# KaHIP/KaMinPar

Measured on NVIDIA H100. Metric: lp_edges_per_second, higher is better.
Workload: dtype int32

## Files before the change

kaminpar_b200/csrc/kmp_lp.cu:

```cuda
#include <cuda_runtime.h>

#include <algorithm>
#include <chrono>
#include <cstdio>
#include <cstring>
#include <new>
#include <string>
#include <vector>

#include <cstdlib>
#include <dlfcn.h>
#include <nccl.h>
#include <cub/device/device_radix_sort.cuh>
#include <cub/device/device_scan.cuh>

#include "../../include/kaminpar_b200_contraction.h"
#include "../../include/kaminpar_b200_lp.h"
#include "lp_commit.cuh"
#include "lp_device.cuh"
#include "lp_lowgroup.cuh"
#include "lp_strict.cuh"
#include "lp_sweep.cuh"

using namespace kmp;
// ... 508 lines not shown
      cudaOccupancyMaxActiveBlocksPerMultiprocessor(&per_sm, kernel, T * TEAMS, smem) != cudaSuccess || per_sm < 1) {
    return false;
  }
  h->team_grid[MODE][EW][P64][team_size_index(T)] = static_cast<uint32_t>(sms * per_sm);
  return true;
}

template <int MODE, bool EW, bool P64> bool configure_team_kernels(kmp_lp_handle *h, int sms) {
  cudaFuncSetAttribute(sweep_hub_scatter<MODE, EW, P64>, cudaFuncAttributeMaxDynamicSharedMemorySize, kHubScatterSmem);
  bool ok = configure_team<MODE, EW, P64, 32, 512, 8, !EW>(h, sms) && configure_team<MODE, EW, P64, 128, 2048, 4>(h, sms) &&
            configure_team<MODE, EW, P64, 512, 8192, 1>(h, sms);
  if constexpr (EW) {
    ok = ok && configure_team<MODE, EW, P64, 1024, 16384, 1>(h, sms);
  } else {
    ok = ok && configure_team<MODE, EW, P64, 1024, 32768, 1, true>(h, sms);
  }
  return ok;
}

template <int MODE, bool EW, bool P64> cudaError_t launch_sweep_t(kmp_lp_handle *h, int tier, const SweepArgs &a) {
  if (a.list_size == 0) {
    return cudaSuccess;
  }
  const uint32_t tgrid = capped(h, grid_for(a.list_size, 256));
  switch (tier) {
  case 0:
    sweep_thread<MODE, EW, P64, 8><<<tgrid, 256, 0, h->sweep_stream>>>(a);
    break;
  case 1:
    sweep_thread<MODE, EW, P64, 16><<<tgrid, 256, 0, h->sweep_stream>>>(a);
    break;
  case 2:
    sweep_thread<MODE, EW, P64, 32><<<tgrid, 256, 0, h->sweep_stream>>>(a);
    break;
  case 3:
    launch_team<MODE, EW, P64, 32, 512, 8, !EW>(h, a);
    break;
  case 4:
    launch_team<MODE, EW, P64, 128, 2048, 4>(h, a);
    break;
  case 5:
    launch_team<MODE, EW, P64, 512, 8192, 1>(h, a);
    break;
  case 6:
    if constexpr (EW) {
      launch_team<MODE, EW, P64, 1024, 16384, 1>(h, a);
    } else {
      launch_team<MODE, EW, P64, 1024, 32768, 1, true>(h, a);
    }
    break;
  default: {
    HubArgs hb{};
    const uint32_t s_idx = h->cur_subround;
    const uint32_t S = h->lists_S;
    const uint32_t first = h->list_off[kHubTier * S + s_idx] - h->list_off[kHubTier * S];
    hb.table_off = h->t4_table_off.p + first;
    hb.g_tab = h->hub_tab.p;
    hb.cursor = h->hub_cursor.p;
    hb.ovf = h->hub_ovf.p;
    hb.ovf_cap = static_cast<uint32_t>(std::min<uint64_t>(h->t4_max_wave_edges, 0xFFFFFFFFull));
    hb.bucket_cap = h->hub_bucket_cap;
    hb.sel_limit = h->hub_sel_limit;
    hb.stage_adjncy = h->adjncy_16b ? 1u : 0u;
    hb.rank = h->rank;
    hb.world = h->world;
    hb.sel_begin = h->t4_sel_begin.p + first;
    hb.hit = h->t4_hit.p + first;
    for (uint32_t w = h->t4_wave_off[s_idx]; w < h->t4_wave_off[s_idx + 1]; ++w) {
      const kmp_lp_handle::HubWave &wv = h->t4_waves[w];
      hb.item_entry = h->t4_item_entry.p + wv.item_lo;
      hb.item_chunk = h->t4_item_chunk.p + wv.item_lo;
      hb.item_u = h->t4_item_u.p + wv.item_lo;
      hb.item_beg = h->t4_item_beg.p + wv.item_lo;
      hb.item_deg = h->t4_item_deg.p + wv.item_lo;
      hb.num_items = wv.item_hi - wv.item_lo;
      hb.queue = h->ctr32.p + 64 + w;
      hb.ovf_count = h->ctr32.p + 512 + w;
      sweep_hub_scatter<MODE, EW, P64><<<capped(h, std::min<uint32_t>(hb.num_items, kSMs * 4)), kHubThreads, kHubScatterSmem, h->sweep_stream>>>(a, hb, h->m);
      hb.sel_entry = h->t4_sel_entry.p + wv.sel_lo;
      hb.sel_piece = h->t4_sel_piece.p + wv.sel_lo;
      hb.num_sel_items = wv.sel_hi - wv.sel_lo;
      hb.part_best = h->t4_part_best.p + (wv.sel_lo - h->t4_sel_off[s_idx]);
      hb.part_fav = h->t4_part_fav.p + (wv.sel_lo - h->t4_sel_off[s_idx]);
      sweep_hub_select<MODE><<<capped(h, std::min<uint32_t>((hb.num_sel_items + kSelWarps - 1) / kSelWarps, kSMs * 6)), kSelWarps * 32, 0, h->sweep_stream>>>(a, hb);
      h->kernel_launches += 2;
    }
    hb.part_best = h->t4_part_best.p;
    hb.part_fav = h->t4_part_fav.p;
    sweep_hub_final<MODE><<<capped(h, grid_for(static_cast<uint64_t>(a.list_size) * 32, 256)), 256, 0, h->sweep_stream>>>(a, hb);
    break;
  }
  }
  return cudaGetLastError();
}

int timed_begin(kmp_lp_handle *h, int tag, cudaStream_t st = nullptr) {
  if (!h->timing) {
    return -1;
  }
  if (st == nullptr) {
    st = h->stream;
  }
  if (h->sweep_events_used == h->sweep_events.size()) {
    cudaEvent_t x, y;
    cudaEventCreate(&x);
    cudaEventCreate(&y);
    h->sweep_events.emplace_back(x, y);
    h->sweep_event_group.push_back(0);
  }
  const int idx = static_cast<int>(h->sweep_events_used++);
  h->sweep_event_group[idx] = tag;
  cudaEventRecord(h->sweep_events[idx].first, st);
  return idx;
}
void timed_end(kmp_lp_handle *h, int idx, cudaStream_t st = nullptr) {
  if (idx >= 0) {
    cudaEventRecord(h->sweep_events[idx].second, st == nullptr ? h->stream : st);
  }
}

cudaError_t launch_sweep(kmp_lp_handle *h, int mode, int tier, const SweepArgs &a_in) {
  if (a_in.list_size == 0) {
    return cudaSuccess;
  }
  SweepArgs a = a_in;
  a.counters = h->ctr64.p + tier;
  a.queue = h->queue.p + static_cast<size_t>(tier) * kNumGroups * h->lists_S + h->cur_sg;
  if (h->sweep_stream == nullptr) {
    h->sweep_stream = h->stream;
  }
  const int ev = timed_begin(h, tier, h->sweep_stream);
  const bool ew = h->adjwgt != nullptr;
  const int variant = (mode << 2) | (ew ? 2 : 0) | (h->p64 ? 1 : 0);
  cudaError_t e;
  switch (variant) {
  case 0: e = launch_sweep_t<0, false, false>(h, tier, a); break;
  case 1: e = launch_sweep_t<0, false, true>(h, tier, a); break;
  case 2: e = launch_sweep_t<0, true, false>(h, tier, a); break;
  case 3: e = launch_sweep_t<0, true, true>(h, tier, a); break;
  case 4: e = launch_sweep_t<1, false, false>(h, tier, a); break;
  case 5: e = launch_sweep_t<1, false, true>(h, tier, a); break;
  case 6: e = launch_sweep_t<1, true, false>(h, tier, a); break;
  default: e = launch_sweep_t<1, true, true>(h, tier, a); break;
  }
  timed_end(h, ev, h->sweep_stream);
  ++h->kernel_launches;
  ++h->sweep_launches;
  ++h->group_launches[tier];
  return e;
}

struct TraceClock {
  bool on = std::getenv("KMP_TRACE") != nullptr;
  std::chrono::steady_clock::time_point t = std::chrono::steady_clock::now();
  void lap(const char *what) {
    if (on) {
      const auto now = std::chrono::steady_clock::now();
      std::fprintf(stderr, "[kmp trace] %-28s %8.3f ms\n", what, std::chrono::duration<double, std::milli>(now - t).count());
      t = now;
    }
  }
};

int ensure_lists(kmp_lp_handle *h) {
  TraceClock tc;
  const uint32_t S = std::max<uint32_t>(1, h->cfg.sync_subrounds);
  if (h->lists_valid && h->lists_S == S && h->lists_G == h->cfg.sync_granule_log2 &&
// ... 1052 lines not shown
  if (mode == 0) {
    cfg->impl = KMP_LP_TWO_PHASE;
    cfg->two_hop_strategy = KMP_TWO_HOP_MATCH_THREADWISE;
    cfg->isolated_nodes_strategy = KMP_ISOLATED_MATCH_DURING_TWO_HOP;
    cfg->sync_commit_passes = 1;
  } else {
    cfg->impl = KMP_LP_SINGLE_PHASE;
    cfg->two_hop_strategy = KMP_TWO_HOP_DISABLE;
    cfg->isolated_nodes_strategy = KMP_ISOLATED_KEEP;
    cfg->sync_commit_passes = 4;
  }
}

int kmp_lp_create(const kmp_lp_config *cfg, kmp_lp_handle **out) {
  if (cfg == nullptr || out == nullptr) {
    return fail(KMP_ERR_INVALID, "null argument");
  }
  int count = 0;
  cudaError_t e = cudaGetDeviceCount(&count);
  if (e != cudaSuccess || count == 0) {
    return fail(KMP_ERR_CUDA, std::string("no CUDA device available (there is no CPU fallback): ") +
                                  cudaGetErrorString(e));
  }
  if (cfg->schedule != KMP_SCHEDULE_SYNC && cfg->schedule != KMP_SCHEDULE_SEQ_STRICT) {
    return fail(KMP_ERR_INVALID, "unknown schedule");
  }
  if (cfg->schedule == KMP_SCHEDULE_SYNC) {
    if (cfg->tie_breaking_strategy == KMP_TIE_GEOMETRIC) {
      return fail(KMP_ERR_UNSUPPORTED, "tie_breaking_strategy GEOMETRIC is order-dependent (lp_clusterer.cc:252-278): "
                                       "use KMP_SCHEDULE_SEQ_STRICT or UNIFORM");
    }
    if (cfg->tie_breaking_strategy != KMP_TIE_UNIFORM) {
      return fail(KMP_ERR_INVALID, "unknown tie_breaking_strategy");
    }
    if (cfg->two_hop_strategy == KMP_TWO_HOP_MATCH || cfg->two_hop_strategy == KMP_TWO_HOP_CLUSTER) {
      return fail(KMP_ERR_UNSUPPORTED, "global two-hop MATCH / CLUSTER (label_propagation.h:1030-1191) is an id-ordered "
                                       "chain: use MATCH_THREADWISE or KMP_SCHEDULE_SEQ_STRICT");
    }

  }
  if (cfg->relabel_before_second_phase != 0) {
    return fail(KMP_ERR_UNSUPPORTED, "relabel_before_second_phase (label_propagation.h:272-319) is not implemented");
  }
  if (cfg->two_hop_strategy < KMP_TWO_HOP_DISABLE || cfg->two_hop_strategy > KMP_TWO_HOP_CLUSTER_THREADWISE ||
      cfg->isolated_nodes_strategy < KMP_ISOLATED_KEEP || cfg->isolated_nodes_strategy > KMP_ISOLATED_CLUSTER_DURING_TWO_HOP ||
      cfg->impl < KMP_LP_SINGLE_PHASE || cfg->impl > KMP_LP_GROWING_HASH_TABLES) {
    return fail(KMP_ERR_INVALID, "unknown two_hop_strategy / isolated_nodes_strategy / impl");
  }
  kmp_lp_handle *h = new (std::nothrow) kmp_lp_handle();
  if (h == nullptr) {
    return fail(KMP_ERR_ALLOC, "out of host memory");
  }
  h->cfg = *cfg;
  if (const char *e = std::getenv("KMP_HUB_BUCKET_CAP")) {
    h->hub_bucket_cap = static_cast<uint32_t>(std::min<long>(kBucketCap, std::max(1, std::atoi(e))));
  }
  if (const char *e = std::getenv("KMP_HUB_SEL_LIMIT")) {
    h->hub_sel_limit = static_cast<uint32_t>(std::max(0, std::atoi(e)));
  }
  if (const char *e = std::getenv("KMP_HUB_WAVE_SLOTS")) {
    h->hub_wave_slots = static_cast<uint64_t>(std::max(32ll, std::atoll(e)));
  }
  if (const char *e = std::getenv("KMP_GRID_CAP")) {
    h->grid_cap = static_cast<uint32_t>(std::max(1, std::atoi(e)));
  }
  if (h->cfg.sync_subrounds == 0) {
    h->cfg.sync_subrounds = 8;
  }
  if (h->cfg.sync_commit_passes == 0) {
    h->cfg.sync_commit_passes = 1;
  }
  int dev = cfg->device;
  if (dev < 0) {
    cudaGetDevice(&dev);
  }
  h->device = dev;
  if (cudaSetDevice(dev) != cudaSuccess || cudaStreamCreateWithFlags(&h->owned_stream, cudaStreamNonBlocking) != cudaSuccess ||
      cudaEventCreate(&h->ev_begin) != cudaSuccess || cudaEventCreate(&h->ev_end) != cudaSuccess) {
    delete h;
    return fail(KMP_ERR_CUDA, "failed to create stream/events");
  }
  h->stream = h->owned_stream;
  h->sweep_stream = h->stream;
  for (int i = 0; i < 3; ++i) {
    if (cudaStreamCreateWithFlags(&h->side_stream[i], cudaStreamNonBlocking) != cudaSuccess ||
        cudaEventCreateWithFlags(&h->ev_join[i], cudaEventDisableTiming) != cudaSuccess) {
      delete h;
      return fail(KMP_ERR_CUDA, "failed to create side streams");
    }
  }
  if (cudaEventCreateWithFlags(&h->ev_fork, cudaEventDisableTiming) != cudaSuccess) {
    delete h;
    return fail(KMP_ERR_CUDA, "failed to create events");
  }
  if (const char *e = std::getenv("KMP_FORCE_P64")) {
    h->force_p64 = std::atoi(e) != 0;
  }
  int sms = kSMs;
  cudaDeviceGetAttribute(&sms, cudaDevAttrMultiProcessorCount, dev);
  int coop = 0, per_sm = 0, per_sm_r = 0;
  cudaDeviceGetAttribute(&coop, cudaDevAttrCooperativeLaunch, dev);
  if (coop == 0) {
    delete h;
    return fail(KMP_ERR_CUDA, "this device does not support cooperative launches");
  }
  if (cudaOccupancyMaxActiveBlocksPerMultiprocessor(&per_sm, commit_cluster_fused<false>, 256, 0) != cudaSuccess ||
      per_sm < 1 ||
      cudaOccupancyMaxActiveBlocksPerMultiprocessor(&per_sm_r, commit_refine_fused<false>, 256, kSmemPrivLimit * 4) !=
          cudaSuccess ||
      per_sm_r < 1) {
    delete h;
    return fail(KMP_ERR_CUDA, "a fused commit kernel cannot be resident on this device");
  }
  if (h->grid_bar.ensure(2) != cudaSuccess || cudaMemset(h->grid_bar.p, 0, 2 * sizeof(unsigned)) != cudaSuccess) {
    delete h;
    return fail(KMP_ERR_CUDA, "failed to allocate the grid barrier");
  }
  h->fused_blocks = sms * per_sm;
  h->fused_blocks_refine = sms * per_sm_r;
  if (!configure_low_groups(h, sms)) {
    delete h;
    return fail(KMP_ERR_CUDA, "a persistent low-degree clustering kernel cannot be resident on this device");
  }
  if (!(configure_team_kernels<0, false, false>(h, sms) && configure_team_kernels<0, false, true>(h, sms) &&
        configure_team_kernels<0, true, false>(h, sms) && configure_team_kernels<0, true, true>(h, sms) &&
        configure_team_kernels<1, false, false>(h, sms) && configure_team_kernels<1, false, true>(h, sms) &&
        configure_team_kernels<1, true, false>(h, sms) && configure_team_kernels<1, true, true>(h, sms))) {
    delete h;
    return fail(KMP_ERR_CUDA, "a sweep_team kernel cannot be resident on this device");
  }
  *out = h;
  return KMP_OK;
}

int kmp_lp_destroy(kmp_lp_handle *h) {
  if (h == nullptr) {
    return KMP_OK;
  }
  cudaSetDevice(h->device);
  cudaStreamSynchronize(h->stream);
  if (h->comm != nullptr) {
    g_nccl.CommDestroy(h->comm);
    h->comm = nullptr;
  }
  kmp_lp_free_scratch(h);
  h->own_xadj.release();
  h->own_adjncy.release();
  h->own_vwgt.release();
  h->own_adjwgt.release();
  h->order.release();
  for (auto &p : h->sweep_events) {
    cudaEventDestroy(p.first);
    cudaEventDestroy(p.second);
  }
  cudaEventDestroy(h->ev_begin);
  cudaEventDestroy(h->ev_end);
  if (h->ev_ct0 != nullptr) {
    cudaEventDestroy(h->ev_ct0);
    cudaEventDestroy(h->ev_ct1);
  }
  cudaEventDestroy(h->ev_fork);
  for (int i = 0; i < 3; ++i) {
    cudaEventDestroy(h->ev_join[i]);
    cudaStreamDestroy(h->side_stream[i]);
  }
  cudaStreamDestroy(h->owned_stream);
  delete h;
  return KMP_OK;
// ... 736 lines not shown
```

kaminpar_b200/csrc/lp_sweep.cuh:

```cuda
#pragma once

#include "lp_device.cuh"
#include "lp_sortnet.cuh"

namespace kmp {

template <int MODE>
__device__ __forceinline__ void emit_proposal(const SweepArgs &a, uint32_t idx, uint32_t u, uint32_t target,
                                              int32_t uw) {
  a.mv_u[idx] = u;
  a.mv_t[idx] = target;
  if (!a.accumulate) {
    return;
  }
  if (MODE == 0) {
    atomicAdd(&a.incoming[target], uw);
  } else {
    const uint32_t lvl = ladder_level(bijective32(u, a.base_commit));
    atomicAdd(&a.hist[target * kLadderLevels + lvl], uw);
  }
}

__device__ __forceinline__ void block_count_flush(const SweepArgs &a, unsigned long long edges,
                                                  unsigned long long nodes) {
// ... 109 lines not shown
      if (top_ok) {
        best = top;
        lazy_done = true;
      }
    }
    if (!lazy_done) {
      int32_t run = 0;
#pragma unroll
      for (int j = 0; j < N; ++j) {
        run += EW ? ws[j] : 1;
        const bool last = (j == N - 1) || (keys[j + 1 < N ? j + 1 : j] != keys[j]);
        if (last) {
          const int32_t rating = run;
          run = 0;
          if (keys[j] != kEmpty) {
            Cand f;
            const Cand c = eval_candidate<MODE>(a, u, own, uw, own_w, keys[j], rating, MODE == 0 ? false : store_fav, f);
            if (cand_better<MODE>(c, best)) {
              best = c;
            }
          }
        }
      }
    }
  }
  return finish_vertex<MODE>(a, u, own, store_fav, best, fav, target);
}

template <int MODE>
__device__ __forceinline__ void emit_cta_iteration(const SweepArgs &a, bool proposes, uint32_t u, uint32_t target,
                                                   int32_t uw, uint32_t it, uint32_t (&s_cnt)[2][8],
                                                   uint32_t (&s_base)[2]) {
  const unsigned ballot = __ballot_sync(kFull, proposes);
  const int lane = threadIdx.x & 31;
  const int wib = threadIdx.x >> 5;
  const int par = it & 1;
  if (lane == 0) {
    s_cnt[par][wib] = static_cast<uint32_t>(__popc(ballot));
  }
  __syncthreads();
  if (threadIdx.x == 0) {
    uint32_t total = 0;
    for (int w = 0; w < 8; ++w) {
      total += s_cnt[par][w];
    }
    s_base[par] = total != 0 ? atomicAdd(a.mover_count, total) : 0u;
  }
  __syncthreads();
  if (proposes) {
    uint32_t idx = s_base[par] + __popc(ballot & ((1u << lane) - 1u));
    for (int w = 0; w < wib; ++w) {
      idx += s_cnt[par][w];
    }
    emit_proposal<MODE>(a, idx, u, target, uw);
  }
}

template <int MODE, bool EW, bool P64, int N> __global__ void __launch_bounds__(256) sweep_thread(const SweepArgs a) {
  __shared__ uint32_t s_cnt[2][8];
  __shared__ uint32_t s_base[2];
  unsigned long long edges = 0, nodes = 0;
  const uint32_t stride = gridDim.x * blockDim.x;
  const uint32_t bound = (a.list_size + 255u) & ~255u;
  uint32_t it = 0;
  for (uint32_t i = blockIdx.x * blockDim.x + threadIdx.x; i < bound; i += stride, ++it) {
    bool proposes = false;
    uint32_t target = 0;
    int32_t uw = 1;
    ThreadRow<0> r;
    r.u = 0;
    if (i < a.list_size) {
      r.u = a.list[i];
      const bool flag = a.active == nullptr || a.active[r.u] != 0;
      if (flag || a.pull) {
        load_row<0>(a, r);
        proposes = sweep_thread_vertex<MODE, EW, P64, N>(a, r, flag, edges, nodes, target, uw);
      }
    }
    emit_cta_iteration<MODE>(a, proposes, r.u, target, uw, it, s_cnt, s_base);
  }
  block_count_flush(a, edges, nodes);
}

__device__ __forceinline__ uint32_t pow2_ceil(uint32_t x) {
  return x <= 1 ? 1u : (1u << (32 - __clz(static_cast<int>(x - 1))));
}

__device__ __forceinline__ void table_add(uint32_t *keys, int32_t *vals, uint32_t mask, bool direct, uint32_t key,
                                          int32_t w) {
  uint32_t slot = direct ? key : (lowbias32(key) & mask);
  while (true) {
    const uint32_t prev = atomicCAS(&keys[slot], kEmpty, key);
    if (prev == kEmpty || prev == key) {
      atomicAdd(&vals[slot], w);
      return;
    }
    slot = (slot + 1) & mask;
  }
}

template <int T> struct TeamSync {
  static __device__ __forceinline__ void sync(int id) {
    if (T == 32) {
      __syncwarp();
    } else {
      asm volatile("bar.sync %0, %1;" ::"r"(id), "r"(T) : "memory");
    }
  }
  static __device__ __forceinline__ bool any(int id, bool p) {
    if (T == 32) {
      __syncwarp();
      return __any_sync(kFull, p);
    } else {
      int r;
      asm volatile(
          "{\n"
          ".reg .pred q, r;\n"
          "setp.ne.s32 q, %3, 0;\n"
          "bar.red.or.pred r, %1, %2, q;\n"
          "selp.s32 %0, 1, 0, r;\n"
          "}\n"
          : "=r"(r)
          : "r"(id), "r"(T), "r"(static_cast<int>(p))
          : "memory");
      return r != 0;
    }
  }
};

template <int MODE, int T>
__device__ __forceinline__ Cand team_argmax(int id, int tid, Cand c, Cand *s_red) {
  Cand r = warp_argmax<MODE>(kFull, c);
  if (T == 32) {
    return r;
  }
  TeamSync<T>::sync(id);
  if ((tid & 31) == 0) {
    s_red[tid >> 5] = r;
  }
  TeamSync<T>::sync(id);
  Cand x = cand_none();
  if ((tid & 31) < T / 32) {
    x = s_red[tid & 31];
  }
  return warp_argmax<MODE>(kFull, x);
}

template <bool V16> struct TeamVals;
template <> struct TeamVals<false> {
  using word = int32_t;
  static constexpr int kBytesPerSlot = 4;
  static __device__ __forceinline__ void add(word *v, uint32_t slot, int32_t w) { atomicAdd(&v[slot], w); }
  static __device__ __forceinline__ int32_t get(const word *v, uint32_t slot) { return v[slot]; }
  static __device__ __forceinline__ void clear(word *v, uint32_t slot) { v[slot] = 0; }
};
template <> struct TeamVals<true> {
  using word = uint32_t;
  static constexpr int kBytesPerSlot = 2;
  static __device__ __forceinline__ void add(word *v, uint32_t slot, int32_t w) {
    atomicAdd(&v[slot >> 1], static_cast<uint32_t>(w) << ((slot & 1u) * 16u));
  }
  static __device__ __forceinline__ int32_t get(const word *v, uint32_t slot) {
    return static_cast<int32_t>((v[slot >> 1] >> ((slot & 1u) * 16u)) & 0xFFFFu);
  }
  static __device__ __forceinline__ void clear(word *v, uint32_t slot) { reinterpret_cast<uint16_t *>(v)[slot] = 0; }
};

template <bool V16, bool EW>
__device__ __forceinline__ bool team_table_add(uint32_t *keys, typename TeamVals<V16>::word *vals, uint32_t mask,
                                               bool direct, uint32_t key, int32_t w, uint32_t &slot) {
  slot = direct ? key : (lowbias32(key) & mask);
  while (true) {
    const uint32_t prev = atomicCAS(&keys[slot], kEmpty, key);
    if (!EW && prev == kEmpty) {
      return true;
    }
    if (prev == kEmpty || prev == key) {
      TeamVals<V16>::add(vals, slot, w);
// ... 185 lines not shown
          Cand cb = cand_none();
          for (uint32_t l0 = 0; l0 < nc; l0 += T * 4) {
            uint32_t kk[4];
            int32_t rr[4], ww[4];
#pragma unroll
            for (int j = 0; j < 4; ++j) {
              const uint32_t l = l0 + j * T + tid;
              const uint32_t s = l < nc ? list[l] : 0u;
              kk[j] = l < nc ? keys[s] : kEmpty;
              rr[j] = l < nc ? team_rating<V16, EW>(vals, s) : 0;
            }
#pragma unroll
            for (int j = 0; j < 4; ++j) {
              ww[j] = kk[j] != kEmpty ? a.weight[kk[j]] : 0;
            }
#pragma unroll
            for (int j = 0; j < 4; ++j) {
              if (kk[j] != kEmpty) {
                Cand ff;
                const Cand cc = eval_candidate_w<0>(a, u, own, uw, own_w, kk[j], rr[j], ww[j], false, ff);
                if (cand_better<0>(cc, cb)) {
                  cb = cc;
                }
              }
            }
          }
          best = team_argmax<0, T>(bar, tid, cb, s_red);
        }
      } else {
        for (uint32_t l = tid; l < nc; l += T) {
          const uint32_t s = list[l];
          const uint32_t k = keys[s];
          Cand ff;
          const Cand cc = eval_candidate_w<1>(a, u, own, uw, own_w, k, team_rating<V16, EW>(vals, s), a.weight[k], false, ff);
          if (cand_better<1>(cc, c)) {
            c = cc;
          }
        }
        best = team_argmax<1, T>(bar, tid, c, s_red);
      }
    }
    for (uint32_t l = tid; l < nc; l += T) {
      const uint32_t s = list[l];
      keys[s] = kEmpty;
      TV::clear(vals, s);
    }
    if (act && tid == 0) {
      if (T == 32) {
        edges += deg;
        nodes += 1;
      } else {
        s_edges[team] += deg;
        s_nodes[team] += 1;
      }
      if (a.active != nullptr && flag) {
        a.active[u] = 0;
      }
      uint32_t target;
      if (finish_vertex<MODE>(a, u, own, store_fav, best, fav, target)) {
        const uint32_t idx = atomicAdd(a.mover_count, 1u);
        emit_proposal<MODE>(a, idx, u, target, uw);
      }
    }
    TeamSync<T>::sync(bar);
  }
  if (T > 32 && tid == 0) {
    edges = s_edges[team];
    nodes = s_nodes[team];
  }
  if (tid == 0 && nodes != 0) {
    atomicAdd(&a.counters[0], edges);
    atomicAdd(&a.counters[kCounterNodesOffset], nodes);
  }
}

constexpr int kChunkEdges = 2048;
constexpr int kSliceEdges = 256;
constexpr int kSliceTableSlots = 512;
constexpr int kChunkThreads = 256;
constexpr uint32_t kBucketCap = 512;
constexpr uint32_t kBucketTargetFill = 256;
constexpr uint32_t kSelTableSlots = 1024;
constexpr int kSelWarps = 4;

struct HubOverflow {
  uint32_t bucket;
  uint32_t key;
  int32_t rating;
  uint32_t pad;
};

struct HubArgs {
  const uint32_t *__restrict__ item_entry;
  const uint32_t *__restrict__ item_chunk;
  const uint32_t *__restrict__ item_u;
  const uint32_t *__restrict__ item_beg;
  const uint32_t *__restrict__ item_deg;
  uint32_t num_items;
  const uint32_t *__restrict__ table_off;
  unsigned long long *__restrict__ g_tab;
  uint32_t *__restrict__ cursor;
  HubOverflow *__restrict__ ovf;
  uint32_t *__restrict__ ovf_count;
  uint32_t ovf_cap;
  uint32_t bucket_cap;
  uint32_t sel_limit;
  uint32_t stage_adjncy;
  const uint32_t *__restrict__ sel_entry;
  const uint32_t *__restrict__ sel_piece;
  uint32_t num_sel_items;
  const uint32_t *__restrict__ sel_begin;
  Cand *__restrict__ part_best;
  Cand *__restrict__ part_fav;
  uint32_t rank, world;
  uint32_t *__restrict__ queue;
  uint32_t *__restrict__ hit;
};

__host__ __device__ __forceinline__ uint32_t hub_buckets(uint32_t full_degree) {
  const uint32_t need = (full_degree + kBucketTargetFill - 1) / kBucketTargetFill;
  uint32_t p = 1;
  while (p < need) {
    p <<= 1;
  }
  return p;
}

__device__ __forceinline__ uint32_t smem_u32(const void *p) {
  return static_cast<uint32_t>(__cvta_generic_to_shared(p));
}
__device__ __forceinline__ void mbar_init(uint64_t *bar, uint32_t count) {
  asm volatile("mbarrier.init.shared::cta.b64 [%0], %1;" ::"r"(smem_u32(bar)), "r"(count) : "memory");
}
__device__ __forceinline__ void mbar_arrive_expect_tx(uint64_t *bar, uint32_t bytes) {
  asm volatile("mbarrier.arrive.expect_tx.shared::cta.b64 _, [%0], %1;" ::"r"(smem_u32(bar)), "r"(bytes) : "memory");
}
__device__ __forceinline__ void mbar_wait(uint64_t *bar, uint32_t parity) {
  asm volatile(
      "{\n"
      ".reg .pred p;\n"
      "WAIT_LOOP:\n"
      "mbarrier.try_wait.parity.shared::cta.b64 p, [%0], %1;\n"
      "@p bra DONE;\n"
      "bra WAIT_LOOP;\n"
      "DONE:\n"
      "}\n" ::"r"(smem_u32(bar)),
      "r"(parity)
      : "memory");
}
__device__ __forceinline__ void tma_load_1d(void *dst_smem, const void *src_gmem, uint32_t bytes, uint64_t *bar) {
  asm volatile("cp.async.bulk.shared::cluster.global.mbarrier::complete_tx::bytes [%0], [%1], %2, [%3];" ::"r"(
                   smem_u32(dst_smem)),
               "l"(src_gmem), "r"(bytes), "r"(smem_u32(bar))
               : "memory");
}

struct HubItem {
  uint32_t valid;
  uint32_t u;
  uint32_t entry;
  uint32_t full_deg;
  uint32_t gbeg, gend;
  uint32_t a0;
  uint32_t staged;
};

__device__ __forceinline__ void mbar_arrive(uint64_t *bar) {
  asm volatile("mbarrier.arrive.shared::cta.b64 _, [%0];" ::"r"(smem_u32(bar)) : "memory");
}

constexpr int kHubStages = 2;
constexpr int kHubConsumerWarps = kChunkThreads / 32;
constexpr int kHubThreads = kChunkThreads + 32;
constexpr int kHubScatterSmem = kHubConsumerWarps * kSliceTableSlots * 8;

template <int MODE, bool EW, bool P64>
__global__ void __launch_bounds__(kHubThreads, 4) sweep_hub_scatter(const SweepArgs a, const HubArgs hb, uint32_t m_total) {
  extern __shared__ __align__(16) unsigned char smem_raw[];
  constexpr int kAllSlots = kHubConsumerWarps * kSliceTableSlots;
  uint32_t *all_keys = reinterpret_cast<uint32_t *>(smem_raw);
  int32_t *all_vals = reinterpret_cast<int32_t *>(smem_raw + sizeof(uint32_t) * kAllSlots);
  __shared__ __align__(16) uint32_t s_adj[kHubStages][kChunkEdges + 8];
  __shared__ __align__(8) uint64_t s_full[kHubStages];
  __shared__ __align__(8) uint64_t s_empty[kHubStages];
  __shared__ HubItem s_item[kHubStages];
  const int lane = threadIdx.x & 31;
  const int wib = threadIdx.x >> 5;
  if (threadIdx.x == 0) {
    for (int s = 0; s < kHubStages; ++s) {
      mbar_init(&s_full[s], 1);
      mbar_init(&s_empty[s], kHubConsumerWarps);
    }
    asm volatile("fence.mbarrier_init.release.cluster;" ::: "memory");
  }
  for (int s = threadIdx.x; s < kAllSlots; s += kHubThreads) {
    all_keys[s] = kEmpty;
    all_vals[s] = 0;
  }
  __syncthreads();

  if (wib == kHubConsumerWarps) {
    if (lane == 0) {
      for (uint32_t k = 0;; ++k) {
        const int stage = static_cast<int>(k % kHubStages);
        const uint32_t round = k / kHubStages;
        mbar_wait(&s_empty[stage], (round & 1u) ^ 1u);
        const uint32_t it = atomicAdd(hb.queue, 1u);
        HubItem d{};
        d.valid = 0;
        if (it >= hb.num_items) {
          d.valid = 2;
          s_item[stage] = d;
          mbar_arrive(&s_full[stage]);
          break;
        }
        const uint32_t entry = hb.item_entry[it];
        const uint32_t u = hb.item_u[it];
        const uint32_t beg0 = hb.item_beg[it];
        const uint32_t full_deg = hb.item_deg[it];
        const uint32_t chunk = hb.item_chunk[it];
        if (entry % hb.world == hb.rank && (a.active == nullptr || a.pull || a.active[u] != 0)) {
          uint32_t deg = full_deg;
          if (deg > a.max_num_neighbors) {
            deg = a.max_num_neighbors;
          }
          const uint32_t cbeg = chunk * kChunkEdges;
          bool ok = cbeg < deg;
          if (ok && MODE == 1) {
            const uint32_t own = a.label[u];
            const int32_t uw = a.vwgt != nullptr ? a.vwgt[u] : 1;
            const int32_t mn = a.min_w != nullptr ? a.min_w[own] : 0;
            ok = !((a.weight[own] - uw) < mn);
          }
          if (ok) {
            const uint32_t cend = (cbeg + kChunkEdges < deg) ? cbeg + kChunkEdges : deg;
            d.valid = 1;
            d.u = u;
            d.entry = entry;
            d.full_deg = full_deg;
            d.gbeg = beg0 + cbeg;
            d.gend = beg0 + cend;
            d.a0 = d.gbeg & ~3u;
            d.staged = 0;
            if (hb.stage_adjncy) {
              uint32_t a1 = (d.gend + 3u) & ~3u;
              const uint32_t m4 = m_total & ~3u;
              if (a1 > m4) {
                a1 = m4;
              }
              d.staged = a1 > d.a0 ? a1 - d.a0 : 0;
            }
          }
        }
        s_item[stage] = d;
        if (d.valid && d.staged > 0) {
          asm volatile("fence.proxy.async.shared::cta;" ::: "memory");
          mbar_arrive_expect_tx(&s_full[stage], d.staged * 4);
          tma_load_1d(&s_adj[stage][0], a.adjncy + d.a0, d.staged * 4, &s_full[stage]);
        } else {
          mbar_arrive(&s_full[stage]);
        }
      }
    }
    return;
  }

  uint32_t *keys = all_keys + wib * kSliceTableSlots;
  int32_t *vals = all_vals + wib * kSliceTableSlots;
  for (uint32_t k = 0;; ++k) {
    const int stage = static_cast<int>(k % kHubStages);
    const uint32_t round = k / kHubStages;
    mbar_wait(&s_full[stage], round & 1u);
    const HubItem d = s_item[stage];
    if (d.valid == 2) {
      break;
    }
    const uint32_t wbeg = d.gbeg + wib * kSliceEdges;
    const bool mine = d.valid && wbeg < d.gend;
    if (mine) {
      const uint32_t wend = wbeg + kSliceEdges < d.gend ? wbeg + kSliceEdges : d.gend;
      const uint32_t staged_end = d.a0 + d.staged;
      bool hit = false;
      for (uint32_t e0 = wbeg; e0 < wend; e0 += 128) {
        uint32_t k4[4];
        int32_t w4[4];
#pragma unroll
        for (int j = 0; j < 4; ++j) {
          const uint32_t e = e0 + j * 32 + lane;
          k4[j] = kEmpty;
          w4[j] = 0;
          if (e < wend) {
            const uint32_t v = e < staged_end ? s_adj[stage][e - d.a0] : a.adjncy[e];
            bool ok = true;
            if (MODE == 1 && a.communities != nullptr) {
              ok = a.communities[d.u] == a.communities[v];
            }
            const typename LabG<P64>::word g = load_labg<P64>(a, v);
            hit = hit || stamp_hit(LabG<P64>::stamp(g), a.window);
            if (ok) {
              k4[j] = LabG<P64>::label(g);
              w4[j] = EW ? a.adjwgt[e] : 1;
            }
          }
        }
#pragma unroll
        for (int j = 0; j < 4; ++j) {
          if (k4[j] != kEmpty) {
            table_add(keys, vals, kSliceTableSlots - 1, false, k4[j], w4[j]);
          }
        }
      }
      if (a.pull && __any_sync(kFull, hit) && lane == 0) {
        atomicOr(&hb.hit[d.entry], 1u);
      }
    }
    __syncwarp();
    if (lane == 0) {
      mbar_arrive(&s_empty[stage]);
    }
    if (mine) {
      const uint32_t pmask = hub_buckets(d.full_deg) - 1;
      const uint32_t bucket0 = hb.table_off[d.entry];
      constexpr int B = 4;
      for (uint32_t s0 = lane; s0 < kSliceTableSlots; s0 += 32 * B) {
        uint32_t kk[B], bb[B], pos[B];
        int32_t rr[B];
#pragma unroll
        for (int j = 0; j < B; ++j) {
          const uint32_t s = s0 + j * 32;
          kk[j] = keys[s];
          rr[j] = vals[s];
          if (kk[j] != kEmpty) {
            keys[s] = kEmpty;
            vals[s] = 0;
          }
        }
#pragma unroll
        for (int j = 0; j < B; ++j) {
          bb[j] = bucket0 + (lowbias32(kk[j]) & pmask);
          pos[j] = kk[j] != kEmpty ? atomicAdd(&hb.cursor[bb[j]], 1u) : 0u;
        }
#pragma unroll
        for (int j = 0; j < B; ++j) {
          if (kk[j] != kEmpty) {
            if (pos[j] < hb.bucket_cap) {
              hb.g_tab[static_cast<size_t>(bb[j]) * kBucketCap + pos[j]] =
                  (static_cast<unsigned long long>(kk[j]) << 32) | static_cast<uint32_t>(rr[j]);
            } else {
              const uint32_t o = atomicAdd(hb.ovf_count, 1u);
              if (o < hb.ovf_cap) {
                hb.ovf[o] = HubOverflow{bb[j], kk[j], rr[j], 0u};
              }
            }
          }
        }
      }
      __syncwarp();
    }
  }
}

template <int MODE> __global__ void __launch_bounds__(kSelWarps * 32) sweep_hub_select(const SweepArgs a, const HubArgs hb) {
  __shared__ uint32_t s_keys[kSelWarps][kSelTableSlots];
  __shared__ int32_t s_vals[kSelWarps][kSelTableSlots];
  __shared__ uint32_t s_claims_all[kSelWarps];
  const int lane = threadIdx.x & 31;
  const int wib = threadIdx.x >> 5;
  uint32_t *keys = s_keys[wib];
  int32_t *vals = s_vals[wib];
  uint32_t *s_claims = &s_claims_all[wib];
  for (uint32_t s = lane; s < kSelTableSlots; s += 32) {
    keys[s] = kEmpty;
    vals[s] = 0;
  }
  if (lane == 0) {
    *s_claims = 0;
  }
  __syncwarp();
  const uint32_t nwarps = gridDim.x * kSelWarps;
  for (uint32_t it = blockIdx.x * kSelWarps + wib; it < hb.num_sel_items; it += nwarps) {
    const uint32_t entry = hb.sel_entry[it];
    const uint32_t u = a.list[entry];
    Cand c = cand_none(), f = cand_none();
    const bool act = (entry % hb.world == hb.rank) && (a.active == nullptr || a.pull || a.active[u] != 0);
    const uint32_t b = hb.table_off[entry] + hb.sel_piece[it];
    const uint32_t appended = act ? __ldcg(&hb.cursor[b]) : 0u;
    if (appended != 0) {
      const uint32_t full_deg = a.xadj[u + 1] - a.xadj[u];
      const uint32_t pbits = 31 - __clz(static_cast<int>(hub_buckets(full_deg)));
      const uint32_t own = a.label[u];
      const int32_t uw = a.vwgt != nullptr ? a.vwgt[u] : 1;
      const int32_t own_w = a.weight[own];
      const bool store_fav = (MODE == 0) && (uw == own_w) && (own_w <= a.max_cluster_weight / 2);
      const uint32_t n_reg = appended < hb.bucket_cap ? appended : hb.bucket_cap;
      const uint32_t n_ovf = appended > hb.bucket_cap ? min(__ldcg(hb.ovf_count), hb.ovf_cap) : 0u;
      uint32_t tcap = pow2_ceil(2 * appended);
      tcap = tcap < 64 ? 64u : tcap > kSelTableSlots ? kSelTableSlots : tcap;
      const uint32_t tmask = tcap - 1;
      const uint32_t full_limit = tcap / 2 + tcap / 8;
      const uint32_t limit = (hb.sel_limit != 0 && hb.sel_limit < full_limit) ? hb.sel_limit : full_limit;
      const unsigned long long *reg = hb.g_tab + static_cast<size_t>(b) * kBucketCap;
      auto insert = [&](uint32_t key, int32_t r) {
        uint32_t slot = lowbias32(key ^ 0x9E3779B9u) & tmask;
        while (true) {
          const uint32_t prev = atomicCAS(&keys[slot], kEmpty, key);
          if (prev == kEmpty) {
            atomicAdd(s_claims, 1u);
          }
          if (prev == kEmpty || prev == key) {
            atomicAdd(&vals[slot], r);
            return;
          }
          slot = (slot + 1) & tmask;
        }
      };
      uint32_t K = 1;
      while (true) {
        c = cand_none();
        f = cand_none();
        bool overflowed = false;
        for (uint32_t cls = 0; cls < K && !overflowed; ++cls) {
          constexpr int B = 4;
          for (uint32_t i0 = 0; i0 < n_reg && !overflowed; i0 += 32 * B) {
            unsigned long long e[B];
#pragma unroll
            for (int j = 0; j < B; ++j) {
              const uint32_t i = i0 + j * 32 + lane;
              e[j] = i < n_reg ? __ldcs(reg + i) : ~0ull;
            }
#pragma unroll
            for (int j = 0; j < B; ++j) {
              const uint32_t key = static_cast<uint32_t>(e[j] >> 32);
              if (key != kEmpty && ((lowbias32(key) >> pbits) & (K - 1)) == cls) {
                insert(key, static_cast<int32_t>(static_cast<uint32_t>(e[j])));
              }
            }
            if (n_ovf != 0) {
              __syncwarp();
              overflowed = *s_claims > limit;
              __syncwarp();
            }
          }
          for (uint32_t i0 = 0; i0 < n_ovf && !overflowed; i0 += 32 * B) {
#pragma unroll
            for (int j = 0; j < B; ++j) {
              const uint32_t i = i0 + j * 32 + lane;
              if (i < n_ovf) {
                const HubOverflow o = hb.ovf[i];
                if (o.bucket == b && ((lowbias32(o.key) >> pbits) & (K - 1)) == cls) {
                  insert(o.key, o.rating);
                }
              }
            }
            __syncwarp();
            overflowed = *s_claims > limit;
            __syncwarp();
          }
          __syncwarp();
          bool lazy_done = false;
          if (MODE == 0 && K == 1 && !overflowed) {
            Cand ct = cand_none();
            for (uint32_t s = lane; s < tcap; s += 32) {
              const uint32_t kx = keys[s];
              if (kx != kEmpty) {
                const int32_t r = vals[s];
                if (r >= ct.gain && r > 0) {
                  const Cand x{r, 0, tie_hash(a.base_tie, u, kx), kx};
                  if (cand_better<0>(x, ct)) {
                    ct = x;
                  }
                }
                if (store_fav && r >= f.gain && r > 0) {
                  const Cand y{r, 0, tie_hash(a.base_fav, u, kx), kx};
                  if (cand_better<0>(y, f)) {
                    f = y;
                  }
                }
              }
            }
            const Cand top = warp_argmax<0>(kFull, ct);
            bool top_ok = true;
            if (top.gain > 0) {
              top_ok = (a.weight[top.key] + uw <= a.max_cluster_weight) || (top.key == own);
              if (a.communities != nullptr) {
                top_ok = top_ok && (a.communities[top.key] == a.communities[own]);
              }
            }
            if (top_ok) {
              c = top;
              lazy_done = true;
            }
          }
          const bool evaluate = !overflowed && !lazy_done;
          for (uint32_t s0 = 0; s0 < tcap; s0 += 32 * B) {
            uint32_t kk[B];
            int32_t rr[B], ww[B];
#pragma unroll
            for (int j = 0; j < B; ++j) {
              const uint32_t s = s0 + j * 32 + lane;
              kk[j] = s < tcap ? keys[s] : kEmpty;
              rr[j] = kk[j] != kEmpty ? vals[s] : 0;
            }
#pragma unroll
            for (int j = 0; j < B; ++j) {
              ww[j] = (kk[j] != kEmpty && evaluate) ? a.weight[kk[j]] : 0;
            }
#pragma unroll
            for (int j = 0; j < B; ++j) {
              if (kk[j] != kEmpty) {
                const uint32_t s = s0 + j * 32 + lane;
                keys[s] = kEmpty;
                vals[s] = 0;
                if (evaluate) {
                  Cand ff;
                  const Cand cc = eval_candidate_w<MODE>(a, u, own, uw, own_w, kk[j], rr[j], ww[j],
                                                         store_fav && !(MODE == 0 && K == 1), ff);
                  if (cand_better<MODE>(cc, c)) {
                    c = cc;
                  }
                  if (MODE == 0 && cand_better<0>(ff, f)) {
                    f = ff;
                  }
                }
              }
            }
          }
          __syncwarp();
          if (lane == 0) {
            *s_claims = 0;
          }
          __syncwarp();
        }
        if (!overflowed) {
          break;
        }
        K <<= 1;
      }
      if (lane == 0) {
        hb.cursor[b] = 0;
      }
    }
    const Cand best = warp_argmax<MODE>(kFull, c);
    const Cand fav = (MODE == 0) ? warp_argmax<0>(kFull, f) : cand_none();
    if (lane == 0) {
      hb.part_best[it] = best;
      hb.part_fav[it] = fav;
    }
  }
}

template <int MODE> __global__ void __launch_bounds__(256) sweep_hub_final(const SweepArgs a, const HubArgs hb) {
  const int lane = threadIdx.x & 31;
  const uint32_t warp = (blockIdx.x * blockDim.x + threadIdx.x) >> 5;
  const uint32_t nwarps = (gridDim.x * blockDim.x) >> 5;
  unsigned long long edges = 0, nodes = 0;
  for (uint32_t i = warp; i < a.list_size; i += nwarps) {
    if (i % hb.world != hb.rank) {
      continue;
    }
    const uint32_t u = a.list[i];
    bool flag = true;
    if (a.active != nullptr) {
      int fl = 0, ht = 0;
      if (lane == 0) {
        fl = static_cast<int>(a.active[u]);
        if (a.pull) {
          ht = static_cast<int>(hb.hit[i]);
          hb.hit[i] = 0;
        }
      }
      fl = __shfl_sync(kFull, fl, 0);
      ht = __shfl_sync(kFull, ht, 0);
      flag = fl != 0;
      if (fl == 0 && ht == 0) {
        continue;
      }
    }
    const uint32_t full_deg = a.xadj[u + 1] - a.xadj[u];
    uint32_t deg = full_deg;
    if (deg > a.max_num_neighbors) {
      deg = a.max_num_neighbors;
    }
    const uint32_t own = a.label[u];
    const int32_t uw = a.vwgt != nullptr ? a.vwgt[u] : 1;
    const int32_t own_w = a.weight[own];
    const uint32_t pieces = hub_buckets(full_deg);
    const uint32_t first = hb.sel_begin[i];
    const bool store_fav = (MODE == 0) && (uw == own_w) && (own_w <= a.max_cluster_weight / 2);
    Cand c = cand_none(), f = cand_none();
    for (uint32_t q = lane; q < pieces; q += 32) {
      const Cand pb = hb.part_best[first + q];
      if (cand_better<MODE>(pb, c)) {
        c = pb;
      }
      if (MODE == 0) {
        const Cand pf = hb.part_fav[first + q];
        if (cand_better<0>(pf, f)) {
          f = pf;
        }
      }
    }
    const Cand best = warp_argmax<MODE>(kFull, c);
    const Cand fav = (MODE == 0) ? warp_argmax<0>(kFull, f) : cand_none();
    if (lane == 0) {
      edges += deg;
      nodes += 1;
      if (a.active != nullptr && flag) {
        a.active[u] = 0;
      }
      uint32_t target;
      if (finish_vertex<MODE>(a, u, own, store_fav, best, fav, target)) {
        const uint32_t idx = atomicAdd(a.mover_count, 1u);
        emit_proposal<MODE>(a, idx, u, target, uw);
      }
// ... 7 lines not shown
```

Baseline: 41.25 billion.

## Track claimed hash slots in per-warp lists to avoid full-table scans in hub kernels

The hub scatter and select kernels now record each newly claimed shared-memory hash slot in a per-warp uint16 list, using ballot and popc. Drain, evaluation and reset then walk only the claimed slots instead of scanning the whole table. The select kernel drops its per-bucket power-of-two table sizing and the shared atomic claim counter in favour of a fixed-size table and a register claim count, and gets a launch bound of 5 CTAs per SM. Side streams are also created with graded priorities. The change adds shared memory for the lists and a fixed table probe range, which could lower occupancy or lengthen probe chains for small buckets.

```diff
diff --git a/kaminpar_b200/csrc/kmp_lp.cu b/kaminpar_b200/csrc/kmp_lp.cu
--- a/kaminpar_b200/csrc/kmp_lp.cu
+++ b/kaminpar_b200/csrc/kmp_lp.cu
@@ -614,7 +614,7 @@
       hb.num_sel_items = wv.sel_hi - wv.sel_lo;
       hb.part_best = h->t4_part_best.p + (wv.sel_lo - h->t4_sel_off[s_idx]);
       hb.part_fav = h->t4_part_fav.p + (wv.sel_lo - h->t4_sel_off[s_idx]);
-      sweep_hub_select<MODE><<<capped(h, std::min<uint32_t>((hb.num_sel_items + kSelWarps - 1) / kSelWarps, kSMs * 6)), kSelWarps * 32, 0, h->sweep_stream>>>(a, hb);
+      sweep_hub_select<MODE><<<capped(h, std::min<uint32_t>((hb.num_sel_items + kSelWarps - 1) / kSelWarps, kSMs * kSelCtasPerSm)), kSelWarps * 32, 0, h->sweep_stream>>>(a, hb);
       h->kernel_launches += 2;
     }
     hb.part_best = h->t4_part_best.p;
@@ -1833,8 +1833,10 @@
   }
   h->stream = h->owned_stream;
   h->sweep_stream = h->stream;
+  int prio_least = 0, prio_greatest = 0;
+  cudaDeviceGetStreamPriorityRange(&prio_least, &prio_greatest);
   for (int i = 0; i < 3; ++i) {
-    if (cudaStreamCreateWithFlags(&h->side_stream[i], cudaStreamNonBlocking) != cudaSuccess ||
+    if (cudaStreamCreateWithPriority(&h->side_stream[i], cudaStreamNonBlocking, std::min(prio_greatest + i, prio_least)) != cudaSuccess ||
         cudaEventCreateWithFlags(&h->ev_join[i], cudaEventDisableTiming) != cudaSuccess) {
       delete h;
       return fail(KMP_ERR_CUDA, "failed to create side streams");
diff --git a/kaminpar_b200/csrc/lp_sweep.cuh b/kaminpar_b200/csrc/lp_sweep.cuh
--- a/kaminpar_b200/csrc/lp_sweep.cuh
+++ b/kaminpar_b200/csrc/lp_sweep.cuh
@@ -215,18 +215,14 @@
   block_count_flush(a, edges, nodes);
 }
 
-__device__ __forceinline__ uint32_t pow2_ceil(uint32_t x) {
-  return x <= 1 ? 1u : (1u << (32 - __clz(static_cast<int>(x - 1))));
-}
-
-__device__ __forceinline__ void table_add(uint32_t *keys, int32_t *vals, uint32_t mask, bool direct, uint32_t key,
-                                          int32_t w) {
-  uint32_t slot = direct ? key : (lowbias32(key) & mask);
+__device__ __forceinline__ bool table_add(uint32_t *keys, int32_t *vals, uint32_t mask, uint32_t key, int32_t w,
+                                          uint32_t &slot) {
+  slot = lowbias32(key) & mask;
   while (true) {
     const uint32_t prev = atomicCAS(&keys[slot], kEmpty, key);
     if (prev == kEmpty || prev == key) {
       atomicAdd(&vals[slot], w);
-      return;
+      return prev == kEmpty;
     }
     slot = (slot + 1) & mask;
   }
@@ -578,6 +574,11 @@
 constexpr uint32_t kBucketTargetFill = 256;
 constexpr uint32_t kSelTableSlots = 1024;
 constexpr int kSelWarps = 4;
+constexpr uint32_t kSelLimit = kSelTableSlots / 2 + kSelTableSlots / 8;
+constexpr uint32_t kSelBatch = 128;
+constexpr uint32_t kSelListCap = kSelLimit + kSelBatch;
+static_assert(kSelListCap < kSelTableSlots && kBucketCap <= kSelListCap, "select claim list / map sizing");
+constexpr int kSelCtasPerSm = 5;
 
 struct HubOverflow {
   uint32_t bucket;
@@ -677,6 +678,7 @@
   uint32_t *all_keys = reinterpret_cast<uint32_t *>(smem_raw);
   int32_t *all_vals = reinterpret_cast<int32_t *>(smem_raw + sizeof(uint32_t) * kAllSlots);
   __shared__ __align__(16) uint32_t s_adj[kHubStages][kChunkEdges + 8];
+  __shared__ uint16_t s_list[kHubConsumerWarps][kSliceEdges];
   __shared__ __align__(8) uint64_t s_full[kHubStages];
   __shared__ __align__(8) uint64_t s_empty[kHubStages];
   __shared__ HubItem s_item[kHubStages];
@@ -763,6 +765,8 @@
 
   uint32_t *keys = all_keys + wib * kSliceTableSlots;
   int32_t *vals = all_vals + wib * kSliceTableSlots;
+  uint16_t *list = s_list[wib];
+  const unsigned below = (1u << lane) - 1u;
   for (uint32_t k = 0;; ++k) {
     const int stage = static_cast<int>(k % kHubStages);
     const uint32_t round = k / kHubStages;
@@ -773,6 +777,7 @@
     }
     const uint32_t wbeg = d.gbeg + wib * kSliceEdges;
     const bool mine = d.valid && wbeg < d.gend;
+    uint32_t claims = 0;
     if (mine) {
       const uint32_t wend = wbeg + kSliceEdges < d.gend ? wbeg + kSliceEdges : d.gend;
       const uint32_t staged_end = d.a0 + d.staged;
@@ -801,9 +806,13 @@
         }
 #pragma unroll
         for (int j = 0; j < 4; ++j) {
-          if (k4[j] != kEmpty) {
-            table_add(keys, vals, kSliceTableSlots - 1, false, k4[j], w4[j]);
-          }
+          uint32_t slot = 0;
+          const unsigned claimed =
+              __ballot_sync(kFull, k4[j] != kEmpty && table_add(keys, vals, kSliceTableSlots - 1, k4[j], w4[j], slot));
+          if ((claimed >> lane) & 1u) {
+            list[claims + __popc(claimed & below)] = static_cast<uint16_t>(slot);
+          }
+          claims += __popc(claimed);
         }
       }
       if (a.pull && __any_sync(kFull, hit) && lane == 0) {
@@ -818,15 +827,18 @@
       const uint32_t pmask = hub_buckets(d.full_deg) - 1;
       const uint32_t bucket0 = hb.table_off[d.entry];
       constexpr int B = 4;
-      for (uint32_t s0 = lane; s0 < kSliceTableSlots; s0 += 32 * B) {
+      for (uint32_t l0 = 0; l0 < claims; l0 += 32 * B) {
         uint32_t kk[B], bb[B], pos[B];
         int32_t rr[B];
 #pragma unroll
         for (int j = 0; j < B; ++j) {
-          const uint32_t s = s0 + j * 32;
-          kk[j] = keys[s];
-          rr[j] = vals[s];
-          if (kk[j] != kEmpty) {
+          const uint32_t l = l0 + j * 32 + lane;
+          kk[j] = kEmpty;
+          rr[j] = 0;
+          if (l < claims) {
+            const uint32_t s = list[l];
+            kk[j] = keys[s];
+            rr[j] = vals[s];
             keys[s] = kEmpty;
             vals[s] = 0;
           }
@@ -856,21 +868,20 @@
   }
 }
 
-template <int MODE> __global__ void __launch_bounds__(kSelWarps * 32) sweep_hub_select(const SweepArgs a, const HubArgs hb) {
+template <int MODE>
+__global__ void __launch_bounds__(kSelWarps * 32, kSelCtasPerSm) sweep_hub_select(const SweepArgs a, const HubArgs hb) {
   __shared__ uint32_t s_keys[kSelWarps][kSelTableSlots];
   __shared__ int32_t s_vals[kSelWarps][kSelTableSlots];
-  __shared__ uint32_t s_claims_all[kSelWarps];
+  __shared__ uint16_t s_list[kSelWarps][kSelListCap];
   const int lane = threadIdx.x & 31;
   const int wib = threadIdx.x >> 5;
+  const unsigned below = (1u << lane) - 1u;
   uint32_t *keys = s_keys[wib];
   int32_t *vals = s_vals[wib];
-  uint32_t *s_claims = &s_claims_all[wib];
+  uint16_t *list = s_list[wib];
   for (uint32_t s = lane; s < kSelTableSlots; s += 32) {
     keys[s] = kEmpty;
     vals[s] = 0;
-  }
-  if (lane == 0) {
-    *s_claims = 0;
   }
   __syncwarp();
   const uint32_t nwarps = gridDim.x * kSelWarps;
@@ -890,34 +901,38 @@
       const bool store_fav = (MODE == 0) && (uw == own_w) && (own_w <= a.max_cluster_weight / 2);
       const uint32_t n_reg = appended < hb.bucket_cap ? appended : hb.bucket_cap;
       const uint32_t n_ovf = appended > hb.bucket_cap ? min(__ldcg(hb.ovf_count), hb.ovf_cap) : 0u;
-      uint32_t tcap = pow2_ceil(2 * appended);
-      tcap = tcap < 64 ? 64u : tcap > kSelTableSlots ? kSelTableSlots : tcap;
-      const uint32_t tmask = tcap - 1;
-      const uint32_t full_limit = tcap / 2 + tcap / 8;
-      const uint32_t limit = (hb.sel_limit != 0 && hb.sel_limit < full_limit) ? hb.sel_limit : full_limit;
+      const uint32_t limit = (hb.sel_limit != 0 && hb.sel_limit < kSelLimit) ? hb.sel_limit : kSelLimit;
       const unsigned long long *reg = hb.g_tab + static_cast<size_t>(b) * kBucketCap;
-      auto insert = [&](uint32_t key, int32_t r) {
-        uint32_t slot = lowbias32(key ^ 0x9E3779B9u) & tmask;
-        while (true) {
-          const uint32_t prev = atomicCAS(&keys[slot], kEmpty, key);
-          if (prev == kEmpty) {
-            atomicAdd(s_claims, 1u);
-          }
-          if (prev == kEmpty || prev == key) {
-            atomicAdd(&vals[slot], r);
-            return;
-          }
-          slot = (slot + 1) & tmask;
-        }
+      uint32_t claims = 0;
+      auto insert = [&](bool pred, uint32_t key, int32_t r) {
+        uint32_t slot = 0;
+        bool mine = false;
+        if (pred) {
+          slot = lowbias32(key ^ 0x9E3779B9u) & (kSelTableSlots - 1);
+          while (true) {
+            const uint32_t prev = atomicCAS(&keys[slot], kEmpty, key);
+            if (prev == kEmpty || prev == key) {
+              atomicAdd(&vals[slot], r);
+              mine = prev == kEmpty;
+              break;
+            }
+            slot = (slot + 1) & (kSelTableSlots - 1);
+          }
+        }
+        const unsigned claimed = __ballot_sync(kFull, mine);
+        if (mine) {
+          list[claims + __popc(claimed & below)] = static_cast<uint16_t>(slot);
+        }
+        claims += __popc(claimed);
       };
+      constexpr int B = kSelBatch / 32;
       uint32_t K = 1;
       while (true) {
         c = cand_none();
         f = cand_none();
         bool overflowed = false;
         for (uint32_t cls = 0; cls < K && !overflowed; ++cls) {
-          constexpr int B = 4;
-          for (uint32_t i0 = 0; i0 < n_reg && !overflowed; i0 += 32 * B) {
+          for (uint32_t i0 = 0; i0 < n_reg && !overflowed; i0 += kSelBatch) {
             unsigned long long e[B];
 #pragma unroll
             for (int j = 0; j < B; ++j) {
@@ -927,50 +942,44 @@
 #pragma unroll
             for (int j = 0; j < B; ++j) {
               const uint32_t key = static_cast<uint32_t>(e[j] >> 32);
-              if (key != kEmpty && ((lowbias32(key) >> pbits) & (K - 1)) == cls) {
-                insert(key, static_cast<int32_t>(static_cast<uint32_t>(e[j])));
-              }
+              insert(key != kEmpty && ((lowbias32(key) >> pbits) & (K - 1)) == cls, key,
+                     static_cast<int32_t>(static_cast<uint32_t>(e[j])));
             }
             if (n_ovf != 0) {
-              __syncwarp();
-              overflowed = *s_claims > limit;
-              __syncwarp();
-            }
-          }
-          for (uint32_t i0 = 0; i0 < n_ovf && !overflowed; i0 += 32 * B) {
+              overflowed = claims > limit;
+            }
+          }
+          for (uint32_t i0 = 0; i0 < n_ovf && !overflowed; i0 += kSelBatch) {
+            HubOverflow o[B];
 #pragma unroll
             for (int j = 0; j < B; ++j) {
               const uint32_t i = i0 + j * 32 + lane;
-              if (i < n_ovf) {
-                const HubOverflow o = hb.ovf[i];
-                if (o.bucket == b && ((lowbias32(o.key) >> pbits) & (K - 1)) == cls) {
-                  insert(o.key, o.rating);
-                }
-              }
-            }
-            __syncwarp();
-            overflowed = *s_claims > limit;
-            __syncwarp();
+              o[j] = i < n_ovf ? hb.ovf[i] : HubOverflow{~0u, kEmpty, 0, 0u};
+            }
+#pragma unroll
+            for (int j = 0; j < B; ++j) {
+              insert(o[j].bucket == b && ((lowbias32(o[j].key) >> pbits) & (K - 1)) == cls, o[j].key, o[j].rating);
+            }
+            overflowed = claims > limit;
           }
           __syncwarp();
           bool lazy_done = false;
           if (MODE == 0 && K == 1 && !overflowed) {
             Cand ct = cand_none();
-            for (uint32_t s = lane; s < tcap; s += 32) {
+            for (uint32_t l = lane; l < claims; l += 32) {
+              const uint32_t s = list[l];
               const uint32_t kx = keys[s];
-              if (kx != kEmpty) {
-                const int32_t r = vals[s];
-                if (r >= ct.gain && r > 0) {
-                  const Cand x{r, 0, tie_hash(a.base_tie, u, kx), kx};
-                  if (cand_better<0>(x, ct)) {
-                    ct = x;
-                  }
+              const int32_t r = vals[s];
+              if (r >= ct.gain && r > 0) {
+                const Cand x{r, 0, tie_hash(a.base_tie, u, kx), kx};
+                if (cand_better<0>(x, ct)) {
+                  ct = x;
                 }
-                if (store_fav && r >= f.gain && r > 0) {
-                  const Cand y{r, 0, tie_hash(a.base_fav, u, kx), kx};
-                  if (cand_better<0>(y, f)) {
-                    f = y;
-                  }
+              }
+              if (store_fav && r >= f.gain && r > 0) {
+                const Cand y{r, 0, tie_hash(a.base_fav, u, kx), kx};
+                if (cand_better<0>(y, f)) {
+                  f = y;
                 }
               }
             }
@@ -988,14 +997,15 @@
             }
           }
           const bool evaluate = !overflowed && !lazy_done;
-          for (uint32_t s0 = 0; s0 < tcap; s0 += 32 * B) {
-            uint32_t kk[B];
+          for (uint32_t l0 = 0; l0 < claims; l0 += 32 * B) {
+            uint32_t ss[B], kk[B];
             int32_t rr[B], ww[B];
 #pragma unroll
             for (int j = 0; j < B; ++j) {
-              const uint32_t s = s0 + j * 32 + lane;
-              kk[j] = s < tcap ? keys[s] : kEmpty;
-              rr[j] = kk[j] != kEmpty ? vals[s] : 0;
+              const uint32_t l = l0 + j * 32 + lane;
+              ss[j] = l < claims ? list[l] : 0u;
+              kk[j] = l < claims ? keys[ss[j]] : kEmpty;
+              rr[j] = l < claims ? vals[ss[j]] : 0;
             }
 #pragma unroll
             for (int j = 0; j < B; ++j) {
@@ -1004,9 +1014,8 @@
 #pragma unroll
             for (int j = 0; j < B; ++j) {
               if (kk[j] != kEmpty) {
-                const uint32_t s = s0 + j * 32 + lane;
-                keys[s] = kEmpty;
-                vals[s] = 0;
+                keys[ss[j]] = kEmpty;
+                vals[ss[j]] = 0;
                 if (evaluate) {
                   Cand ff;
                   const Cand cc = eval_candidate_w<MODE>(a, u, own, uw, own_w, kk[j], rr[j], ww[j],
@@ -1022,10 +1031,7 @@
             }
           }
           __syncwarp();
-          if (lane == 0) {
-            *s_claims = 0;
-          }
-          __syncwarp();
+          claims = 0;
         }
         if (!overflowed) {
           break;
```

After: 42.39 billion, median of 6. 1.03x the previous value.
